# skovaka/UNCALLED

Measured on AMD Instinct MI355X. Metric: reads_mapped_per_sec, higher is better.
Workload: dtype u64+f32/f64; 1 GPU; E. coli 4.6 Mb synthetic ref (ecoli_syn seed 1), synthetic r9.4.1 reads (3600 bases ~ 32k samples, 10% off-target), all reference defaults; batches_in_flight=2, remapped_reads=0, parallelism=reads sharded over 1 GPU(s), index replicated

## Files before the change

### uncalled_amd/csrc/k_map.hip

```cpp
#include <hip/hip_runtime.h>

#include <type_traits>

#include "fm_dev.h"
#include "unc_dev_types.h"
#include "wave_prims.h"


#include "map_lds.h"
#include "map_sched.h"
#include "map_tracker.h"
#include "map_sort.h"
#include "map_sort_wide.h"

namespace unc {

__device__ __forceinline__ uint32_t float_orderable(float f) {
    uint32_t u = __float_as_uint(f);
    return (u & 0x80000000u) ? ~u : (u | 0x80000000u);
}

struct ChildHdr { uint32_t moves, meta; float seed_prob, last; uint64_t hist; };
__device__ __forceinline__ ChildHdr make_child(uint32_t pmoves, uint32_t pmeta, float last, float subc, uint64_t hist, uint64_t s, uint64_t e,
                                               uint32_t kmer, float prob, uint32_t move, uint32_t p_seed_len, float p_min_seed_prob,
// ... 12 lines not shown
    if (full) moves |= PATH_TAIL_MOVE;
    c.moves = moves;
    c.meta = kmer | (len << META_LEN_SHIFT) | (cstay << META_STAY_SHIFT) | (pmeta & META_SA_CHECKED) |
             ((!full && len == (uint32_t)SEED_LEN) ? META_FIRST_FULL : 0u);
    c.hist = move ? (hist & 0x3FFull) | ((((hist >> 10) << 2) | (kmer & 3u)) << 10) : hist;
    const uint32_t move_count = (uint32_t)__popc(moves);
    const bool seed_ok = len == p_seed_len && c.seed_prob >= p_min_seed_prob && s == e && (moves & 1u) == 1u &&
                         (float)(len - move_count) <= p_max_stay;
    key.a = key_len_bits ? ((((s << key_len_bits) | (e - s)) << 16) | child_idx) : ((s << KEY_LEN_BITS) | (e - s));
    key.b = ((uint64_t)float_orderable(c.seed_prob) << 32) | ((uint64_t)child_idx << 16) | (move_count << KEYB_MOVES_SHIFT) |
            (seed_ok ? KEYB_SEED_FLAG : 0u) | kmer;
    return c;
}

template <bool NARROW>
__device__ __forceinline__ void write_source(gptr_t buf, uint32_t idx, uint64_t s, uint64_t e, uint32_t kmer, float prob) {
    const uint32_t o = idx << PATH_SHIFT;
    const uint64_t r = NARROW ? (s | (e << 32)) : ((s << KEY_LEN_BITS) | (e - s));
    gst(buf, o, make_uint4((uint32_t)r, (uint32_t)(r >> 32), 1u, kmer | (1u << META_LEN_SHIFT)));
    gst(buf, o + 16u, make_uint4(__float_as_uint(prob), 0u, kmer, 0u));
}


#ifndef UNC_LB
#define UNC_LB 4
#endif

typedef const UNC_AS_CONST MapArgs *kargs_t;

struct WaveCtx {
    uint32_t event_i, n_parents, cur, n_surv_par;
    uint32_t tstatus;
    uint32_t nchild, n_seedp;
    uint32_t mixed;
    uint32_t kl;
    uint32_t scnt[6];
    uint32_t n_surv, n_src;
    uint32_t conf;
    uint32_t par_unsorted;
    uint32_t walked;
    uint32_t notes;
    uint32_t flags_save[NKMER / 32];
};
__shared__ WaveCtx s_w;
__shared__ Tracker s_T;
__shared__ uint64_t s_cyc[12];

__device__ __forceinline__ uint32_t ctx_get(const uint32_t &f) { return uniform32(f); }
#define CTX_SET(field, v) do { if (lane == 0) s_w.field = (v); } while (0)

#ifndef UNC_PROF_SORT
#define UNC_PROF_SORT 0
#endif
template <bool PROF> struct PhaseClock {
    uint64_t tk;
    __device__ __forceinline__ PhaseClock() : tk(PROF ? (uint64_t)clock64() : 0ull) {}
    __device__ __forceinline__ void reset() { if constexpr (PROF) tk = (uint64_t)clock64(); }
    __device__ __forceinline__ void end(int i, int lane) {
        if constexpr (PROF) {
            if ((UNC_PROF_SORT || UNC_DBG_SEED) && i >= 8) i = 1;
            const uint64_t tn = (uint64_t)clock64();
            if (lane == 0) s_cyc[i] += tn - tk;
            tk = tn;
        }
    }
};
#if UNC_PROF_SORT
struct SortClock {
    uint64_t tk;
    __device__ __forceinline__ SortClock() : tk((uint64_t)clock64()) {}
    __device__ __forceinline__ void end(int i, int lane) {
        const uint64_t tn = (uint64_t)clock64();
        if (lane == 0) { s_cyc[i] += tn - tk; s_cyc[2] -= tn - tk; }
        tk = tn;
    }
};
#else
struct SortClock { __device__ __forceinline__ void end(int, int) {} };
#endif

__device__ __forceinline__ TrackerMem tracker_mem(kargs_t A, gptr_t sb) {
    TrackerMem M;
    M.sb = sb; M.off_heads = A->sc.off_cl_dir; M.off_chunks = A->sc.off_cl_chunks;
    M.max_nodes = A->sc.max_clusters / 4 ? A->sc.max_clusters / 4 : 1u;
    M.n_buckets = A->ix.n_buckets; M.shift = A->ix.bucket_shift;
    M.pool.nodes = (gptr_t)A->pool.nodes;
    M.pool.q = A->pool.q; M.pool.cells = A->pool.cells; M.pool.cap_mask = A->pool.cap_mask;
    return M;
}

static __device__ __noinline__ void phase_P(kargs_t A_, float level, int lane) {
    const kargs_t A = uniform_ptr(A_);
    const UNC_AS_GLOBAL float4 *const model4 = (const UNC_AS_GLOBAL float4 *)A->ix.model4;
#pragma unroll 4
    for (int j = 0; j < NKMER / WAVE; ++j) {
        const uint32_t k = (uint32_t)j * WAVE + (uint32_t)lane;
        const float4 row = g_load(model4 + k);
        const float mu = row.x, v2 = row.y, ld = row.z;
        const float d = __fsub_rn(level, mu);
        const double q = -((double)d * (double)d) / (double)v2;
        s_probs[k] = (float)(q - (double)ld);
    }
    wave_sync();
}

struct FmView {
    const UNC_AS_GLOBAL uint32_t *bwt;
    const UNC_AS_GLOBAL uint32_t *fm32;
    const UNC_AS_GLOBAL uint64_t *sa, *sa_dense;
    const UNC_AS_CONST uint64_t *L2;
    uint64_t primary, seq_len;
};
__device__ __forceinline__ FmView fm_view(kargs_t A) {
// ... 252 lines not shown
        for (uint32_t l0 = 0; l0 < nwrite; l0 += WAVE) {
            const uint32_t li = l0 + (uint32_t)lane;
            if (li < nwrite) {
                const uint32_t d = s_cdesc[li];
                const uint32_t pl = d & 63u, type = (d >> 6) & 7u, ci = (pl << 2) | ((type - 1u) & 3u);
                const uint32_t pmt = s_pmeta[pl], pmv = s_pmoves[pl];
                const float last = s_plast[pl], subc = s_psubc[pl];
                const uint64_t hist = s_phist[pl];
                const uint32_t pk = pmt & META_KMER_MASK;
                Row cs, ce;
                uint32_t ck, mv;
                if (type == 0) { cs = s_pstart[pl]; ce = s_pend[pl]; ck = pk; mv = 0; }
                else {
                    const uint64_t pr = s_res[ci];
                    if constexpr (NARROW) { cs = (uint32_t)pr; ce = cs + (uint32_t)(pr >> 32) - 1u; }
                    else { cs = pr >> RES_BITS; ce = cs + (pr & ((1ull << RES_BITS) - 1ull)) - 1ull; }
                    ck = ((pk << 2) & KMASK) | (type - 1u); mv = 1;
                }
                SortKey key;
                const uint32_t gi = nchild + li;
                const ChildHdr c = make_child(pmv, pmt, last, subc, hist, cs, ce, ck, s_probs[ck], mv, p_seed_len, p_min_seed_prob, p_max_stay, gi, klb, key);
                const uint32_t co = chd_off + (gi << PATH_SHIFT);
                if constexpr (NARROW) gst(sb, co, make_uint4(cs, ce, c.moves, c.meta));
                else { const uint64_t r = (cs << KEY_LEN_BITS) | (ce - cs); gst(sb, co, make_uint4((uint32_t)r, (uint32_t)(r >> 32), c.moves, c.meta)); }
                gst(sb, co + 16u, make_uint4(__float_as_uint(c.last), __float_as_uint(subc), (uint32_t)c.hist, (uint32_t)(c.hist >> 32)));
                if constexpr (NARROW) {
                    const uint32_t run = (d >> 9) ? 5u : type;
                    gst(sb, str_off + run * run_bytes + ((uint32_t)s_ckpos[li] << 3), key.a);
                    gst(sb, info_off + (gi << 3), key.b);
                } else {
                    const bool csrc = base + pl >= n_surv_par;
                    const uint64_t wm = type == 0u ? wm0 : type == 1u ? wm1 : type == 2u ? wm2 : type == 3u ? wm3 : wm4;
                    const uint32_t ws = type == 0u ? ws0 : type == 1u ? ws1 : type == 2u ? ws2 : type == 3u ? ws3 : ws4;
                    const uint32_t kpos = csrc ? wsx + (li - w_src_cpos0) : ws + (uint32_t)__popcll(wm & ((1ull << pl) - 1ull));
                    gst(sb, str_off + (csrc ? 5u : type) * (run_bytes << 1) + (kpos << 4), key);
                }
            }
        }
        nchild += nwrite;
        wave_sync();
        clk.end(11, lane);
    }
    clk.end(1, lane);
    uint32_t tst = 0;
    if (n_seedp > max_seed_paths) { tst = UNC_READ_SEED_OVERFLOW; n_seedp = max_seed_paths; }
    if (lane == 0) {
        s_w.nchild = nchild; s_w.n_seedp = n_seedp; s_w.tstatus |= tst; s_w.par_unsorted = par_bad ? 1u : 0u;
        s_w.scnt[0] = scnt0; s_w.scnt[1] = scnt1; s_w.scnt[2] = scnt2; s_w.scnt[3] = scnt3; s_w.scnt[4] = scnt4; s_w.scnt[5] = scntx;
    }
    wave_sync();
    return c_nbr;
}

static __device__ __noinline__ void merge_walk(kargs_t A_, gptr_t sb_, KeyArr<1> KA_, KeyArr<4> KB_, int lane);
static __device__ __noinline__ void merge_walk_w(kargs_t A_, gptr_t sb_, KeyArr<1> KA_, KeyArr<4> KB_, int lane);

template <bool NARROW>
static __device__ __noinline__ void phase_S(kargs_t A_, gptr_t sb_, int lane) {
    const kargs_t A = uniform_ptr(A_);
    const gptr_t sb = uniform_ptr(sb_);
    const uint32_t n = ctx_get(s_w.nchild);
    const uint32_t max_paths = A->sc.max_paths;
    const uint32_t ukeys_off = A->sc.off_keys, skeys_off = A->sc.off_keys + A->sc.keys_cap * (uint32_t)sizeof(SortKey);
    UNC_AS_GLOBAL SortKey *const ukeys = reinterpret_cast<UNC_AS_GLOBAL SortKey *>(sb + ukeys_off);
    UNC_AS_GLOBAL SortKey *const skeys = reinterpret_cast<UNC_AS_GLOBAL SortKey *>(sb + skeys_off);
    uint32_t kl = NARROW ? A->ix.key_len_bits : 0u;
    if (lane == 0) { s_w.walked = 0u; s_w.mixed = 0u; }
    if constexpr (NARROW) {
        const uint32_t str_off = A->sc.off_streams, sk_off = skeys_off, run_bytes = max_paths << 3;
        uint32_t scnt0 = ctx_get(s_w.scnt[0]), scnt1 = ctx_get(s_w.scnt[1]), scnt2 = ctx_get(s_w.scnt[2]), scnt3 = ctx_get(s_w.scnt[3]),
                 scnt4 = ctx_get(s_w.scnt[4]), nx = ctx_get(s_w.scnt[5]);
#ifdef LANESIM
        {
            const uint32_t cnt[6] = {scnt0, scnt1, scnt2, scnt3, scnt4, nx};
            uint32_t tot = 0;
            for (uint32_t r = 0; r < 6; ++r) {
                tot += cnt[r];
                for (uint32_t i = (uint32_t)lane; i < cnt[r]; i += WAVE)
                    UNC_SIM_CHECK((gld<uint64_t>(sb, str_off + r * run_bytes + (i << 3)) & 0xFFFFu) < n);
            }
            UNC_SIM_CHECK(tot == n);
        }
#endif
        if (n > MERGE_MIN && !ctx_get(s_w.par_unsorted)) {
            const uint32_t x_off = str_off + 5u * run_bytes;
            uint32_t nviol = 0;
            SortClock sclk;
            if (scnt1 > 1 || scnt2 > 1 || scnt3 > 1 || scnt4 > 1) {
                const uint64_t v4 = repair_runs4(sb, str_off, run_bytes, scnt1, scnt2, scnt3, scnt4, x_off, nx, lane);
                const uint32_t v1 = (uint32_t)v4 & 0xFFFFu, v2 = (uint32_t)(v4 >> 16) & 0xFFFFu, v3 = (uint32_t)(v4 >> 32) & 0xFFFFu, v4r = (uint32_t)(v4 >> 48);
                nviol = v1 + v2 + v3 + v4r;
                if constexpr (MERGE_REPAIR) { scnt1 -= v1; scnt2 -= v2; scnt3 -= v3; scnt4 -= v4r; nx += nviol; }
            }
            wave_sync();
            sclk.end(8, lane);
            if (MERGE_REPAIR || nviol == 0) {
                if (nx > 1) {
                    KeyArr<6> KX;
#pragma unroll
                    for (int r = 0; r < 6; ++r) { KX.adj[r] = x_off; KX.cum[r] = 0; }
                    KX.n = nx;
                    sort_any64(sb, KX, x_off, lane);
                    wave_sync();
                }
                sclk.end(9, lane);
                KeyArr<4> KM;
                KM.cum[0] = 0; KM.cum[1] = scnt1; KM.cum[2] = scnt1 + scnt2; KM.cum[3] = scnt1 + scnt2 + scnt3;
                KM.n = KM.cum[3] + scnt4;
#pragma unroll
                for (uint32_t r = 0; r < 4; ++r) KM.adj[r] = str_off + (r + 1u) * run_bytes - (KM.cum[r] << 3);
                KeyArr<4> KB = KM;
                if (nx > 0) {
                    if (KM.n > 0) {
                        merge_runs<4, 1>(sb, KM, ka_single(x_off, nx), A->sc.off_tmp, lane, 0u);
                        wave_sync();
                        KB.adj[0] = A->sc.off_tmp;
                    } else KB.adj[0] = x_off;
                    KB.cum[1] = KB.cum[2] = KB.cum[3] = KB.n = KM.n + nx;
                    KB.adj[1] = KB.adj[2] = KB.adj[3] = KB.adj[0];
                }
                sclk.end(10, lane);
                merge_walk(A, sb, ka_single(str_off, scnt0), KB, lane);
                CTX_SET(kl, kl);
                CTX_SET(walked, 1u);
                wave_sync();
                sclk.end(11, lane);
                return;
            }
        }
        {
            KeyArr<6> K6;
            const uint32_t c[6] = {scnt0, scnt1, scnt2, scnt3, scnt4, nx};
            uint32_t cum = 0;
#pragma unroll
            for (uint32_t r = 0; r < 6; ++r) { K6.cum[r] = cum; K6.adj[r] = str_off + r * run_bytes - (cum << 3); cum += c[r]; }
            K6.n = cum;
            sort_any64(sb, K6, sk_off, lane);
        }
    }
    if constexpr (!NARROW) {
        const uint32_t str_off = A->sc.off_streams, run_bytes = max_paths << 4;
        uint32_t scnt0 = ctx_get(s_w.scnt[0]), scnt1 = ctx_get(s_w.scnt[1]), scnt2 = ctx_get(s_w.scnt[2]), scnt3 = ctx_get(s_w.scnt[3]),
                 scnt4 = ctx_get(s_w.scnt[4]), nx = ctx_get(s_w.scnt[5]);
        const uint32_t x_off = str_off + 5u * run_bytes;
        if (n > MERGE_MIN && !ctx_get(s_w.par_unsorted)) {
            if (scnt1 > 1) { const uint32_t v = repairw_run(sb, str_off + run_bytes, scnt1, x_off, nx, lane); scnt1 -= v; nx += v; }
            if (scnt2 > 1) { const uint32_t v = repairw_run(sb, str_off + 2u * run_bytes, scnt2, x_off, nx, lane); scnt2 -= v; nx += v; }
            if (scnt3 > 1) { const uint32_t v = repairw_run(sb, str_off + 3u * run_bytes, scnt3, x_off, nx, lane); scnt3 -= v; nx += v; }
            if (scnt4 > 1) { const uint32_t v = repairw_run(sb, str_off + 4u * run_bytes, scnt4, x_off, nx, lane); scnt4 -= v; nx += v; }
            wave_sync();
            uint32_t xs_off = x_off;
            if (nx > 1) {
                const UNC_AS_GLOBAL SortKey *const xin = reinterpret_cast<const UNC_AS_GLOBAL SortKey *>(sb + x_off);
                if (nx <= 64) sort_regs<1>(xin, skeys, nx, lane);
                else if (nx <= 128) sort_regs<2>(xin, skeys, nx, lane);
                else if (nx <= 256) sort_regs<4>(xin, skeys, nx, lane);
                else if (nx <= 512) sort_regs<8>(xin, skeys, nx, lane);
                else sort_hybrid(xin, skeys, nx, lane);
                xs_off = skeys_off;
                wave_sync();
            }
            KeyArr<4> KM;
            KM.cum[0] = 0; KM.cum[1] = scnt1; KM.cum[2] = scnt1 + scnt2; KM.cum[3] = scnt1 + scnt2 + scnt3;
            KM.n = KM.cum[3] + scnt4;
#pragma unroll
            for (uint32_t r = 0; r < 4; ++r) KM.adj[r] = str_off + (r + 1u) * run_bytes - (KM.cum[r] << 4);
            KeyArr<4> KB = KM;
            if (nx > 0) {
                if (KM.n > 0) {
                    mergew_runs<4, 1>(sb, KM, kaw_single(xs_off, nx), ukeys_off, lane);
                    wave_sync();
                    KB.adj[0] = ukeys_off;
                } else KB.adj[0] = xs_off;
                KB.cum[1] = KB.cum[2] = KB.cum[3] = KB.n = KM.n + nx;
                KB.adj[1] = KB.adj[2] = KB.adj[3] = KB.adj[0];
// ... 179 lines not shown
        kq0 = (uint32_t)lane < n ? k0 : ~0ull; kq1 = (uint32_t)lane + WAVE < n ? k1 : ~0ull;
        const uint32_t km0 = (uint32_t)(bq0 & META_KMER_MASK);
        krq = g_load(reinterpret_cast<const UNC_AS_GLOBAL u32x4_t *>(kmer_ranges2) + (s_probs[km0] >= source_prob ? km0 : 0u));
    }
    for (uint32_t base = 0; base < n; base += WAVE) {
        const uint32_t i = base + (uint32_t)lane;
        const bool have = i < n;
        const bool has_next = i + 1 < n;
        const uint32_t nv = n - base < WAVE ? n - base : WAVE;
        Row start, end, nstart;
        uint64_t sbw;
        uint32_t kmer, nkmer;
        bool dup;
        ulonglong2 krc = make_ulonglong2(1ull, 0ull);
        uint32_t kq2i = 0;
        if (kl) {
            const uint64_t ki = kq0, bi = bq0;
            uint64_t kn = (uint64_t)__shfl((unsigned long long)ki, (lane + 1) & 63);
            uint64_t bn = (uint64_t)__shfl((unsigned long long)bi, (lane + 1) & 63);
            const uint64_t kf = bcast64(kq1, 0), bf = bcast64(bq1, 0);
            if (lane == WAVE - 1) { kn = kf; bn = bf; }
            kq0 = kq1; bq0 = bq1;
            {
                const uint64_t k2 = skeys64[i + 2 * WAVE < n ? i + 2 * WAVE : n - 1u];
                kq1 = i + 2 * WAVE < n ? k2 : ~0ull;
                kq2i = (uint32_t)(k2 & 0xFFFFu);
            }
            u32x4_t kt = krq;
            mem_retire(kt);
            krc.x = ((uint64_t)kt.y << 32) | kt.x; krc.y = ((uint64_t)kt.w << 32) | kt.z;
            {
                const uint32_t kmn = (uint32_t)(bq0 & META_KMER_MASK);
                krq = g_load(reinterpret_cast<const UNC_AS_GLOBAL u32x4_t *>(kmer_ranges2) + (s_probs[kmn] >= source_prob ? kmn : 0u));
            }
            walk_decode_narrow<NARROW>(S, kl, ki, kn, bi, bn, have, has_next, nv, lane, start, end, nstart, kmer, nkmer, dup, sbw);
        } else {
            SortKey ki, kn;
            ki.a = ~0ull; ki.b = 0; kn.a = ~0ull; kn.b = ~0ull;
            if (have) ki = g_load(skeys + i);
            if (has_next) kn = g_load(skeys + i + 1);
            start = (Row)(ki.a >> KEY_LEN_BITS); end = start + (Row)(ki.a & KEY_LEN_MASK);
            nstart = (Row)(kn.a >> KEY_LEN_BITS);
            kmer = have ? (uint32_t)(ki.b & META_KMER_MASK) : NKMER + 1u;
            nkmer = has_next ? (uint32_t)(kn.b & META_KMER_MASK) : NKMER + 2u;
            dup = has_next && kn.a == ki.a;
            sbw = ki.b;
        }
        walk_core<NARROW>(C, S, have, has_next, start, end, nstart, kmer, nkmer, dup, sbw, kl != 0, krc, nv, lane);
        if (kl) bq1 = infow[kq2i];
    }
    walk_finish<NARROW>(C, S, lane);
}

static __device__ __noinline__ void merge_walk(kargs_t A_, gptr_t sb_, KeyArr<1> KA_, KeyArr<4> KB_, int lane) {
    const kargs_t A = uniform_ptr(A_);
    const gptr_t sb = uniform_ptr(sb_);
    uint64_t *const s_tile = s_e;
    const KeyArr<1> KA = ka_uniform(KA_);
    const KeyArr<4> KB = ka_uniform(KB_);
    const uint32_t n = KA.n + KB.n;
    const WalkConst<true> C = walk_const<true>(A, sb);
    WalkState<true> S;
    S.n_seedp = ctx_get(s_w.n_seedp);
    walk_begin_narrow(lane);
    const uint32_t kl = A->ix.key_len_bits;
    const float source_prob = C.source_prob;
    const UNC_AS_GLOBAL ulonglong2 *const kmer_ranges2 = (const UNC_AS_GLOBAL ulonglong2 *)A->ix.kmer_ranges;
    const UNC_AS_GLOBAL uint64_t *const infow = reinterpret_cast<const UNC_AS_GLOBAL uint64_t *>(sb + A->sc.off_info);
    uint32_t a0 = 0, b0 = 0;
    uint64_t pend_key = 0;
    bool have_pend = false, bad = false;
    for (uint32_t o0 = 0; o0 < n; o0 += MERGE_TILE) {
        const uint32_t d1 = o0 + MERGE_TILE < n ? o0 + MERGE_TILE : n;
        const bool last_tile = d1 == n;
        const uint32_t a1 = last_tile ? KA.n : merge_split(sb, KA, KB, d1, lane);
        const uint32_t b1 = d1 - a1;
        const uint32_t na = a1 - a0, nb = b1 - b0, tn = na + nb;
        stage_tile(sb, KA, KB, a0, b0, na, tn, s_tile, lane);
        wave_sync();
        const uint32_t d = (uint32_t)lane * MERGE_C < tn ? (uint32_t)lane * MERGE_C : tn;
        const uint32_t cnt = tn - d < MERGE_C ? tn - d : MERGE_C;
        uint32_t lo = d > nb ? d - nb : 0u, hi = d < na ? d : na;
        while (__any(lo < hi)) {
            if (lo < hi) {
                const uint32_t mid = (lo + hi) >> 1;
                if (s_tile[mslot(mid)] < s_tile[mslot(na + d - 1u - mid)]) lo = mid + 1u; else hi = mid;
            }
        }
        uint32_t ia = lo, ib = d - lo;
        uint64_t va = ia < na ? s_tile[mslot(ia)] : ~0ull, vb = ib < nb ? s_tile[mslot(na + ib)] : ~0ull;
        uint64_t o[MERGE_C];
#pragma unroll
        for (uint32_t c = 0; c < MERGE_C; ++c) {
            const bool ta = va < vb;
            o[c] = ta ? va : vb;
            if (ta) ++ia; else ++ib;
            const uint32_t idx = ta ? ia : na + ib;
            const bool ok = ta ? ia < na : ib < nb;
            uint64_t x = ~0ull;
            if (ok && c + 1u < cnt) x = s_tile[mslot(idx)];
            if (ta) va = x; else vb = x;
        }
        {
            uint64_t last = o[0];
            bool w = false;
#pragma unroll
            for (uint32_t c = 1; c < MERGE_C; ++c)
                if (c < cnt) { w = w || !(o[c] > last); last = o[c]; }
            uint64_t pl = (uint64_t)__shfl_up((unsigned long long)last, 1);
            if (lane == 0) pl = pend_key;
            if (cnt > 0 && !(o[0] > pl)) w = true;
            if (__any(w)) bad = true;
        }
        wave_sync();
#pragma unroll
        for (uint32_t c = 0; c < MERGE_C; ++c)
            if (c < cnt) s_tile[mslot(1u + d + c)] = o[c];
        if (lane == 0 && have_pend) s_tile[mslot(0)] = pend_key;
        wave_sync();
#ifdef LANESIM
        for (uint32_t q = 1u + (uint32_t)lane; q <= tn; q += WAVE) {
            const uint64_t kq = s_tile[mslot(q)];
            UNC_SIM_CHECK((kq & 0xFFFFu) < n);
            UNC_SIM_CHECK(((infow[kq & 0xFFFFu] >> 16) & 0xFFFFu) == (kq & 0xFFFFu));
        }
        wave_sync();
#endif
        const uint32_t p0 = have_pend ? 0u : 1u, p1 = last_tile ? tn + 1u : tn;
        uint64_t bq0, bq1;
        {
            const uint32_t pa = p0 + (uint32_t)lane, pb = pa + WAVE;
            bq0 = infow[s_tile[mslot(pa <= tn ? pa : tn)] & 0xFFFFu];
            bq1 = infow[s_tile[mslot(pb <= tn ? pb : tn)] & 0xFFFFu];
        }
        u32x4_t krq;
        {
            const uint32_t km0 = (uint32_t)(bq0 & META_KMER_MASK);
            krq = g_load(reinterpret_cast<const UNC_AS_GLOBAL u32x4_t *>(kmer_ranges2) + (s_probs[km0] >= source_prob ? km0 : 0u));
        }
        for (uint32_t base = p0; base < p1; base += WAVE) {
            const uint32_t p = base + (uint32_t)lane;
            const bool have = p < p1;
            const bool has_next = have && p < tn;
            const uint32_t nv = p1 - base < WAVE ? p1 - base : WAVE;
            const uint64_t bq2 = infow[s_tile[mslot(p + 2 * WAVE <= tn ? p + 2 * WAVE : tn)] & 0xFFFFu];
            const uint64_t ki = have ? s_tile[mslot(p)] : ~0ull, kn = has_next ? s_tile[mslot(p + 1u)] : ~0ull;
            const uint64_t bi = bq0;
            uint64_t bn = (uint64_t)__shfl((unsigned long long)bi, (lane + 1) & 63);
            const uint64_t bf = bcast64(bq1, 0);
            if (lane == WAVE - 1) bn = bf;
            bq0 = bq1;
            u32x4_t kt = krq;
            mem_retire(kt);
            ulonglong2 krc;
            krc.x = ((uint64_t)kt.y << 32) | kt.x; krc.y = ((uint64_t)kt.w << 32) | kt.z;
            {
                const uint32_t kmn = (uint32_t)(bq0 & META_KMER_MASK);
                krq = g_load(reinterpret_cast<const UNC_AS_GLOBAL u32x4_t *>(kmer_ranges2) + (s_probs[kmn] >= source_prob ? kmn : 0u));
            }
            uint32_t start, end, nstart, kmer, nkmer;
            uint64_t sbw;
            bool dup;
            walk_decode_narrow<true>(S, kl, ki, kn, bi, bn, have, has_next, nv, lane, start, end, nstart, kmer, nkmer, dup, sbw);
            walk_core<true>(C, S, have, has_next, start, end, nstart, kmer, nkmer, dup, sbw, true, krc, nv, lane);
            bq1 = bq2;
        }
        pend_key = uniform64(s_tile[mslot(tn)]);
        have_pend = true;
        a0 = a1; b0 = b1;
        wave_sync();
    }
    if (bad && lane == 0) s_w.tstatus |= UNC_READ_SORT_FAULT;
    walk_finish<true>(C, S, lane);
}

static __device__ __noinline__ void merge_walk_w(kargs_t A_, gptr_t sb_, KeyArr<1> KA_, KeyArr<4> KB_, int lane) {
    const kargs_t A = uniform_ptr(A_);
    const gptr_t sb = uniform_ptr(sb_);
    SortKey *const tile = reinterpret_cast<SortKey *>(s_e);
    const KeyArr<1> KA = ka_uniform(KA_);
    const KeyArr<4> KB = ka_uniform(KB_);
    const uint32_t n = KA.n + KB.n;
    const WalkConst<false> C = walk_const<false>(A, sb);
    WalkState<false> S;
    S.n_seedp = ctx_get(s_w.n_seedp);
    uint32_t a0 = 0, b0 = 0;
    SortKey pend_key; pend_key.a = 0; pend_key.b = 0;
    bool have_pend = false, bad = false;
    for (uint32_t o0 = 0; o0 < n; o0 += MERGEW_TILE) {
        const uint32_t d1 = o0 + MERGEW_TILE < n ? o0 + MERGEW_TILE : n;
        const bool last_tile = d1 == n;
        const uint32_t a1 = last_tile ? KA.n : mergew_split(sb, KA, KB, d1, lane);
        const uint32_t b1 = d1 - a1;
        const uint32_t na = a1 - a0, nb = b1 - b0, tn = na + nb;
        stagew_tile(sb, KA, KB, a0, b0, na, tn, tile, lane);
        wave_sync();
        SortKey o[MERGEW_C];
        uint32_t d, cnt;
        mergew_tile(tile, na, nb, lane, o, d, cnt);
        {
            SortKey last = o[0];
            bool w = false;
#pragma unroll
            for (uint32_t c = 1; c < MERGEW_C; ++c)
                if (c < cnt) { w = w || !wk_lt(last, o[c]); last = o[c]; }
            SortKey pl;
            pl.a = (uint64_t)__shfl_up((unsigned long long)last.a, 1); pl.b = (uint64_t)__shfl_up((unsigned long long)last.b, 1);
            if (lane == 0) pl = pend_key;
            if (cnt > 0 && !wk_lt(pl, o[0])) w = true;
            if (__any(w)) bad = true;
        }
        wave_sync();
#pragma unroll
        for (uint32_t c = 0; c < MERGEW_C; ++c)
            if (c < cnt) tile[1u + d + c] = o[c];
        if (lane == 0 && have_pend) tile[0] = pend_key;
        wave_sync();
        const uint32_t p0 = have_pend ? 0u : 1u, p1 = last_tile ? tn + 1u : tn;
        const UNC_AS_GLOBAL ulonglong2 *const kmer_ranges2 = (const UNC_AS_GLOBAL ulonglong2 *)A->ix.kmer_ranges;
        ulonglong2 krq;
        {
            const uint32_t pa = p0 + (uint32_t)lane;
            const uint32_t km0 = (uint32_t)(tile[pa <= tn ? pa : tn].b & META_KMER_MASK);
            krq = g_load(kmer_ranges2 + (s_probs[km0] >= C.source_prob ? km0 : 0u));
        }
// ... 1179 lines not shown
    else hipLaunchKernelGGL((k_map<false, false>), dim3(grid), dim3(WAVE), 0, st, a);
}
__global__ void k_sched_init(DevSched S) {
    const uint32_t t = blockIdx.x * blockDim.x + threadIdx.x, cap = S.cap_mask + 1u;
    const uint32_t part = t / cap, i = t % cap, spp = S.n_slots / S.n_parts;
    if (part < S.n_parts) {
        SchedCell f; f.seq = i < spp ? i + 1u : i; f.val = part * spp + i;
        S.free_cells[t] = f;
        SchedCell p; p.seq = i; p.val = 0;
        S.park_cells[t] = p;
    }
    if (t == 0) {
        SchedCtl c;
        memset(&c, 0, sizeof c);
        for (uint32_t q = 0; q < S.n_parts; ++q) c.freeq[q].tail = spp;
        *S.ctl = c;
    }
}
void launch_sched_init(const DevSched &S, hipStream_t st) {
    const uint32_t n = (S.cap_mask + 1u) * S.n_parts;
    hipLaunchKernelGGL(k_sched_init, dim3((n + 255) / 256), dim3(256), 0, st, S);
}
__global__ void k_xcd_probe(uint32_t *out) { if (threadIdx.x == 0) out[blockIdx.x] = xcd_id(); }
void launch_xcd_probe(uint32_t *out, uint32_t n_blocks, hipStream_t st) { hipLaunchKernelGGL(k_xcd_probe, dim3(n_blocks), dim3(64), 0, st, out); }
__global__ void k_pool_init(DevPool B) {
    const uint32_t i = blockIdx.x * blockDim.x + threadIdx.x, cap = B.cap_mask + 1u;
    if (i < cap) {
        SchedCell f; f.seq = i < B.n_chunks ? i + 1u : i; f.val = i;
        B.cells[i] = f;
    }
    if (i == 0) {
        PoolQueue q;
        memset(&q, 0, sizeof q);
        q.avail = (int32_t)B.n_chunks;
        q.tail = B.n_chunks;
        q.low_water = B.n_chunks;
        *B.q = q;
    }
}
void launch_pool_init(const DevPool &B, hipStream_t st) {
    const uint32_t cap = B.cap_mask + 1u;
    hipLaunchKernelGGL(k_pool_init, dim3((cap + 255) / 256), dim3(256), 0, st, B);
}
uint32_t map_kernel_waves_per_cu() { return 4 * UNC_LB; }
int map_kernel_attributes(bool narrow, bool profile, uint32_t *out4) {
    hipFuncAttributes a;
    const void *f = narrow ? (profile ? (const void *)k_map<true, true> : (const void *)k_map<false, true>)
                           : (profile ? (const void *)k_map<true, false> : (const void *)k_map<false, false>);
    const hipError_t e = hipFuncGetAttributes(&a, f);
    if (e != hipSuccess) return (int)e;
    out4[0] = (uint32_t)a.numRegs; out4[1] = (uint32_t)a.localSizeBytes; out4[2] = (uint32_t)a.sharedSizeBytes; out4[3] = (uint32_t)a.maxThreadsPerBlock;
    return 0;
}
}
```

### uncalled_amd/csrc/map_sort.h

```cpp
#pragma once

namespace unc {


__device__ __forceinline__ bool key_gt(uint64_t a1, uint64_t b1, uint64_t a2, uint64_t b2) {
    return a1 > a2 || (a1 == a2 && b1 > b2);
}

template <int E>
__device__ __forceinline__ void merge_stages(uint64_t (&a)[E], uint64_t (&b)[E], uint32_t base, uint32_t k, uint32_t j_from,
                                             int lane) {
    for (uint32_t j = j_from; j > 0; j >>= 1) {
        if (j >= (uint32_t)E) {
            const uint32_t d = j / (uint32_t)E;
            const bool lower = ((uint32_t)lane & d) == 0;
#pragma unroll
            for (int e = 0; e < E; ++e) {
                uint64_t pa = xor_lane64(a[e], d);
                uint64_t pb = xor_lane64(b[e], d);
                uint32_t p = base + (uint32_t)lane * E + (uint32_t)e;
                bool up = (p & k) == 0;
                bool want_min = lower == up;
                bool gt = key_gt(a[e], b[e], pa, pb);
                if (want_min ? gt : !gt) { a[e] = pa; b[e] = pb; }
// ... 289 lines not shown
static __device__ __noinline__ void sort_any64(gptr_t sb, KeyArr<6> K, uint32_t out_off, int lane) {
    const uint32_t n = uniform32(K.n);
    if (n <= 64) sort_regs64<1>(sb, K, out_off, lane);
    else if (n <= 128) sort_regs64<2>(sb, K, out_off, lane);
    else if (n <= 256) sort_regs64<4>(sb, K, out_off, lane);
    else if (n <= 512) sort_regs64<8>(sb, K, out_off, lane);
    else sort_hybrid64(sb, K, out_off, lane);
}

constexpr uint32_t MERGE_MIN = 256;
#ifndef UNC_MERGE_REPAIR
#define UNC_MERGE_REPAIR 1
#endif
constexpr bool MERGE_REPAIR = UNC_MERGE_REPAIR != 0;
constexpr uint32_t MERGE_C = 9;
constexpr uint32_t MERGE_TILE = MERGE_C * WAVE;
__device__ __forceinline__ uint32_t mslot(uint32_t i) { return i + (i >> 3); }
constexpr uint32_t MERGE_LDS_KEYS = MERGE_TILE + MERGE_TILE / 8 + 1;
static_assert(MERGE_LDS_KEYS <= S_E_WORDS && NKMER * 4 <= S_E_WORDS * 8, "merge tile / source list must fit the staging buffer");

constexpr uint32_t SPLIT_PROBES = 16;
template <int RA, int RB>
__device__ __forceinline__ uint32_t merge_split(cgptr_t sb, const KeyArr<RA> &A, const KeyArr<RB> &B, uint32_t d, int lane) {
    uint32_t lo = d > B.n ? d - B.n : 0u, hi = d < A.n ? d : A.n;
    while (lo < hi) {
        const uint32_t span = hi - lo, step = (span + SPLIT_PROBES - 1u) / SPLIT_PROBES;
        const uint32_t p = lo + (uint32_t)lane * step;
        bool less = false;
        if ((uint32_t)lane < SPLIT_PROBES && p < hi) less = ka_load(sb, A, p) < ka_load(sb, B, d - 1u - p);
        const uint32_t c = (uint32_t)__popcll(__ballot(less));
        const uint32_t nlo = c ? lo + (c - 1u) * step + 1u : lo;
        const uint32_t nhi = lo + c * step < hi ? lo + c * step : hi;
        lo = nlo; hi = c ? nhi : lo;
    }
    return lo;
}

template <int RA, int RB>
__device__ __forceinline__ void stage_tile(cgptr_t sb, const KeyArr<RA> &A, const KeyArr<RB> &B, uint32_t a0, uint32_t b0, uint32_t na, uint32_t tn,
                                           uint64_t *s_tile, int lane) {
    uint64_t v[MERGE_C];
#pragma unroll
    for (uint32_t c = 0; c < MERGE_C; ++c) {
        const uint32_t i0 = (uint32_t)lane + c * WAVE, i = i0 < tn ? i0 : tn - 1u;
        const uint32_t ja = a0 + i, jb = b0 + (i - na);
        const uint32_t off = i < na ? ka_adj(A, ja) + (ja << 3) : ka_adj(B, jb) + (jb << 3);
        v[c] = gld<uint64_t>(sb, off);
    }
#pragma unroll
    for (uint32_t c = 0; c < MERGE_C; ++c) {
        const uint32_t i = (uint32_t)lane + c * WAVE;
        if (i < tn) s_tile[mslot(i)] = v[c];
    }
}

template <int RA, int RB>
static __device__ __noinline__ uint32_t merge_runs(gptr_t sb_, KeyArr<RA> A_, KeyArr<RB> B_, uint32_t out_off_, int lane, uint32_t verify_) {
    const gptr_t sb = uniform_ptr(sb_);
    uint64_t *const s_tile = s_e;
    const KeyArr<RA> A = ka_uniform(A_);
    const KeyArr<RB> B = ka_uniform(B_);
    const uint32_t out_off = uniform32(out_off_), verify = uniform32(verify_);
    const uint32_t n = A.n + B.n;
    uint32_t a0 = 0, b0 = 0;
    uint64_t prev_last = 0;
    bool bad = false;
    for (uint32_t o0 = 0; o0 < n; o0 += MERGE_TILE) {
        const uint32_t d1 = o0 + MERGE_TILE < n ? o0 + MERGE_TILE : n;
        const uint32_t a1 = d1 == n ? A.n : merge_split(sb, A, B, d1, lane);
        const uint32_t b1 = d1 - a1;
        const uint32_t na = a1 - a0, nb = b1 - b0, tn = na + nb;
        stage_tile(sb, A, B, a0, b0, na, tn, s_tile, lane);
        wave_sync();
        const uint32_t d = (uint32_t)lane * MERGE_C < tn ? (uint32_t)lane * MERGE_C : tn;
        const uint32_t cnt = tn - d < MERGE_C ? tn - d : MERGE_C;
        uint32_t lo = d > nb ? d - nb : 0u, hi = d < na ? d : na;
        while (__any(lo < hi)) {
            if (lo < hi) {
                const uint32_t mid = (lo + hi) >> 1;
                if (s_tile[mslot(mid)] < s_tile[mslot(na + d - 1u - mid)]) lo = mid + 1u; else hi = mid;
            }
        }
        uint32_t ia = lo, ib = d - lo;
        uint64_t va = ia < na ? s_tile[mslot(ia)] : ~0ull, vb = ib < nb ? s_tile[mslot(na + ib)] : ~0ull;
        uint64_t o[MERGE_C];
#pragma unroll
        for (uint32_t c = 0; c < MERGE_C; ++c) {
            const bool ta = va < vb;
            o[c] = ta ? va : vb;
            if (ta) ++ia; else ++ib;
            const uint32_t idx = ta ? ia : na + ib;
            const bool ok = ta ? ia < na : ib < nb;
            uint64_t x = ~0ull;
            if (ok && c + 1u < cnt) x = s_tile[mslot(idx)];
            if (ta) va = x; else vb = x;
        }
        wave_sync();
#pragma unroll
        for (uint32_t c = 0; c < MERGE_C; ++c)
            if (c < cnt) s_tile[mslot(d + c)] = o[c];
        wave_sync();
#pragma unroll
        for (uint32_t c = 0; c < MERGE_C; ++c) {
            const uint32_t i = (uint32_t)lane + c * WAVE;
            if (i < tn) gst(sb, out_off + ((o0 + i) << 3), s_tile[mslot(i)]);
        }
// ... 114 lines not shown
```

Measured before the change: 25170 reads/s.

## Fold small extra-key run into merge-walk as a three-way in-register merge

When the unsorted extra-key run has at most a wavefront's worth of keys, it is now loaded into registers, sorted with a single in-wave bitonic sort, and merged tile-by-tile into the merge walk. Previously it was sorted in global scratch and merged into the four repaired runs through a separate merge_runs pass into temporary storage. This removes a global sort and a full merge pass over the four runs for the common case. The cost is a second in-tile merge and extra LDS syncs on tiles that absorb extra keys, plus some added register pressure in merge_walk. Larger extra runs keep the old path.

```diff
diff --git a/uncalled_amd/csrc/k_map.hip b/uncalled_amd/csrc/k_map.hip
--- a/uncalled_amd/csrc/k_map.hip
+++ b/uncalled_amd/csrc/k_map.hip
@@ -88,13 +88,16 @@
 #ifndef UNC_PROF_SORT
 #define UNC_PROF_SORT 0
 #endif
+#ifndef UNC_DBG_NX
+#define UNC_DBG_NX 0
+#endif
 template <bool PROF> struct PhaseClock {
     uint64_t tk;
     __device__ __forceinline__ PhaseClock() : tk(PROF ? (uint64_t)clock64() : 0ull) {}
     __device__ __forceinline__ void reset() { if constexpr (PROF) tk = (uint64_t)clock64(); }
     __device__ __forceinline__ void end(int i, int lane) {
         if constexpr (PROF) {
-            if ((UNC_PROF_SORT || UNC_DBG_SEED) && i >= 8) i = 1;
+            if ((UNC_PROF_SORT || UNC_DBG_NX || UNC_DBG_SEED) && i >= 8) i = 1;
             const uint64_t tn = (uint64_t)clock64();
             if (lane == 0) s_cyc[i] += tn - tk;
             tk = tn;
@@ -453,7 +456,14 @@
     return c_nbr;
 }
 
-static __device__ __noinline__ void merge_walk(kargs_t A_, gptr_t sb_, KeyArr<1> KA_, KeyArr<4> KB_, int lane);
+static __device__ __noinline__ void merge_walk(kargs_t A_, gptr_t sb_, KeyArr<1> KA_, KeyArr<4> KB_, uint32_t x_off_, uint32_t nx_, int lane);
+
+#ifdef LANESIM
+extern "C" { unsigned long long unc_sim_merge3_count = 0, unc_sim_merge2_count = 0, unc_sim_merge_nx_hist[MERGE_XCAP + 3] = {0}; }
+#define UNC_SIM_COUNT(c) do { if (lane == 0) __atomic_fetch_add(&(c), 1ull, __ATOMIC_RELAXED); } while (0)
+#else
+#define UNC_SIM_COUNT(c) ((void)0)
+#endif
 static __device__ __noinline__ void merge_walk_w(kargs_t A_, gptr_t sb_, KeyArr<1> KA_, KeyArr<4> KB_, int lane);
 
 template <bool NARROW>
@@ -495,23 +505,30 @@
             }
             wave_sync();
             sclk.end(8, lane);
+#if UNC_DBG_NX
+            if (lane == 0 && (MERGE_REPAIR || nviol == 0)) { s_cyc[8] += 1u; s_cyc[9] += nx <= 64u; s_cyc[10] += nx <= 128u; s_cyc[11] += nviol; }
+#endif
             if (MERGE_REPAIR || nviol == 0) {
-                if (nx > 1) {
+                KeyArr<4> KM;
+                KM.cum[0] = 0; KM.cum[1] = scnt1; KM.cum[2] = scnt1 + scnt2; KM.cum[3] = scnt1 + scnt2 + scnt3;
+                KM.n = KM.cum[3] + scnt4;
+#pragma unroll
+                for (uint32_t r = 0; r < 4; ++r) KM.adj[r] = str_off + (r + 1u) * run_bytes - (KM.cum[r] << 3);
+                if (nx <= MERGE_XCAP) {
+                    UNC_SIM_COUNT(unc_sim_merge3_count);
+                    UNC_SIM_COUNT(unc_sim_merge_nx_hist[nx]);
+                    merge_walk(A, sb, ka_single(str_off, scnt0), KM, x_off, nx, lane);
+                } else {
+                    UNC_SIM_COUNT(unc_sim_merge2_count);
+                    UNC_SIM_COUNT(unc_sim_merge_nx_hist[nx < MERGE_XCAP + 2u ? nx : MERGE_XCAP + 2u]);
                     KeyArr<6> KX;
 #pragma unroll
                     for (int r = 0; r < 6; ++r) { KX.adj[r] = x_off; KX.cum[r] = 0; }
                     KX.n = nx;
                     sort_any64(sb, KX, x_off, lane);
                     wave_sync();
-                }
-                sclk.end(9, lane);
-                KeyArr<4> KM;
-                KM.cum[0] = 0; KM.cum[1] = scnt1; KM.cum[2] = scnt1 + scnt2; KM.cum[3] = scnt1 + scnt2 + scnt3;
-                KM.n = KM.cum[3] + scnt4;
-#pragma unroll
-                for (uint32_t r = 0; r < 4; ++r) KM.adj[r] = str_off + (r + 1u) * run_bytes - (KM.cum[r] << 3);
-                KeyArr<4> KB = KM;
-                if (nx > 0) {
+                    sclk.end(9, lane);
+                    KeyArr<4> KB = KM;
                     if (KM.n > 0) {
                         merge_runs<4, 1>(sb, KM, ka_single(x_off, nx), A->sc.off_tmp, lane, 0u);
                         wave_sync();
@@ -519,9 +536,9 @@
                     } else KB.adj[0] = x_off;
                     KB.cum[1] = KB.cum[2] = KB.cum[3] = KB.n = KM.n + nx;
                     KB.adj[1] = KB.adj[2] = KB.adj[3] = KB.adj[0];
-                }
-                sclk.end(10, lane);
-                merge_walk(A, sb, ka_single(str_off, scnt0), KB, lane);
+                    sclk.end(10, lane);
+                    merge_walk(A, sb, ka_single(str_off, scnt0), KB, x_off, 0u, lane);
+                }
                 CTX_SET(kl, kl);
                 CTX_SET(walked, 1u);
                 wave_sync();
@@ -807,13 +824,15 @@
     walk_finish<NARROW>(C, S, lane);
 }
 
-static __device__ __noinline__ void merge_walk(kargs_t A_, gptr_t sb_, KeyArr<1> KA_, KeyArr<4> KB_, int lane) {
+static __device__ __noinline__ void merge_walk(kargs_t A_, gptr_t sb_, KeyArr<1> KA_, KeyArr<4> KB_, uint32_t x_off_, uint32_t nx_, int lane) {
     const kargs_t A = uniform_ptr(A_);
     const gptr_t sb = uniform_ptr(sb_);
     uint64_t *const s_tile = s_e;
     const KeyArr<1> KA = ka_uniform(KA_);
     const KeyArr<4> KB = ka_uniform(KB_);
-    const uint32_t n = KA.n + KB.n;
+    const uint32_t nx = uniform32(nx_);
+    const uint32_t n2 = KA.n + KB.n;
+    const uint64_t xk = merge3_load_x(sb, uniform32(x_off_), nx, lane);
     const WalkConst<true> C = walk_const<true>(A, sb);
     WalkState<true> S;
     S.n_seedp = ctx_get(s_w.n_seedp);
@@ -822,61 +841,15 @@
     const float source_prob = C.source_prob;
     const UNC_AS_GLOBAL ulonglong2 *const kmer_ranges2 = (const UNC_AS_GLOBAL ulonglong2 *)A->ix.kmer_ranges;
     const UNC_AS_GLOBAL uint64_t *const infow = reinterpret_cast<const UNC_AS_GLOBAL uint64_t *>(sb + A->sc.off_info);
-    uint32_t a0 = 0, b0 = 0;
-    uint64_t pend_key = 0;
-    bool have_pend = false, bad = false;
-    for (uint32_t o0 = 0; o0 < n; o0 += MERGE_TILE) {
-        const uint32_t d1 = o0 + MERGE_TILE < n ? o0 + MERGE_TILE : n;
-        const bool last_tile = d1 == n;
-        const uint32_t a1 = last_tile ? KA.n : merge_split(sb, KA, KB, d1, lane);
-        const uint32_t b1 = d1 - a1;
-        const uint32_t na = a1 - a0, nb = b1 - b0, tn = na + nb;
-        stage_tile(sb, KA, KB, a0, b0, na, tn, s_tile, lane);
-        wave_sync();
-        const uint32_t d = (uint32_t)lane * MERGE_C < tn ? (uint32_t)lane * MERGE_C : tn;
-        const uint32_t cnt = tn - d < MERGE_C ? tn - d : MERGE_C;
-        uint32_t lo = d > nb ? d - nb : 0u, hi = d < na ? d : na;
-        while (__any(lo < hi)) {
-            if (lo < hi) {
-                const uint32_t mid = (lo + hi) >> 1;
-                if (s_tile[mslot(mid)] < s_tile[mslot(na + d - 1u - mid)]) lo = mid + 1u; else hi = mid;
-            }
-        }
-        uint32_t ia = lo, ib = d - lo;
-        uint64_t va = ia < na ? s_tile[mslot(ia)] : ~0ull, vb = ib < nb ? s_tile[mslot(na + ib)] : ~0ull;
-        uint64_t o[MERGE_C];
-#pragma unroll
-        for (uint32_t c = 0; c < MERGE_C; ++c) {
-            const bool ta = va < vb;
-            o[c] = ta ? va : vb;
-            if (ta) ++ia; else ++ib;
-            const uint32_t idx = ta ? ia : na + ib;
-            const bool ok = ta ? ia < na : ib < nb;
-            uint64_t x = ~0ull;
-            if (ok && c + 1u < cnt) x = s_tile[mslot(idx)];
-            if (ta) va = x; else vb = x;
-        }
-        {
-            uint64_t last = o[0];
-            bool w = false;
-#pragma unroll
-            for (uint32_t c = 1; c < MERGE_C; ++c)
-                if (c < cnt) { w = w || !(o[c] > last); last = o[c]; }
-            uint64_t pl = (uint64_t)__shfl_up((unsigned long long)last, 1);
-            if (lane == 0) pl = pend_key;
-            if (cnt > 0 && !(o[0] > pl)) w = true;
-            if (__any(w)) bad = true;
-        }
-        wave_sync();
-#pragma unroll
-        for (uint32_t c = 0; c < MERGE_C; ++c)
-            if (c < cnt) s_tile[mslot(1u + d + c)] = o[c];
-        if (lane == 0 && have_pend) s_tile[mslot(0)] = pend_key;
-        wave_sync();
+    Merge3 M;
+    while (M.o0 < n2) {
+        const bool have_pend = M.have_pend;
+        const uint32_t tn = merge3_tile(sb, KA, KB, nx, xk, M, s_tile, lane);
+        const bool last_tile = M.last_tile;
 #ifdef LANESIM
         for (uint32_t q = 1u + (uint32_t)lane; q <= tn; q += WAVE) {
             const uint64_t kq = s_tile[mslot(q)];
-            UNC_SIM_CHECK((kq & 0xFFFFu) < n);
+            UNC_SIM_CHECK((kq & 0xFFFFu) < n2 + nx);
             UNC_SIM_CHECK(((infow[kq & 0xFFFFu] >> 16) & 0xFFFFu) == (kq & 0xFFFFu));
         }
         wave_sync();
@@ -920,12 +893,10 @@
             walk_core<true>(C, S, have, has_next, start, end, nstart, kmer, nkmer, dup, sbw, true, krc, nv, lane);
             bq1 = bq2;
         }
-        pend_key = uniform64(s_tile[mslot(tn)]);
-        have_pend = true;
-        a0 = a1; b0 = b1;
-        wave_sync();
-    }
-    if (bad && lane == 0) s_w.tstatus |= UNC_READ_SORT_FAULT;
+        merge3_done(M, tn, s_tile);
+    }
+    UNC_SIM_CHECK(M.xc == nx);
+    if (M.bad && lane == 0) s_w.tstatus |= UNC_READ_SORT_FAULT;
     walk_finish<true>(C, S, lane);
 }
 
@@ -2211,4 +2182,37 @@
     out4[0] = (uint32_t)a.numRegs; out4[1] = (uint32_t)a.localSizeBytes; out4[2] = (uint32_t)a.sharedSizeBytes; out4[3] = (uint32_t)a.maxThreadsPerBlock;
     return 0;
 }
-}
+
+#ifdef LANESIM
+__global__ void k_sim_merge3(char *buf, uint32_t run_keys, const uint32_t *cnt, uint64_t *out, uint32_t *tiles) {
+    const int lane = lane_id();
+    const gptr_t sb = (gptr_t)buf;
+    const uint32_t run_bytes = run_keys << 3, nx = cnt[5];
+    KeyArr<4> KM;
+    KM.cum[0] = 0; KM.cum[1] = cnt[1]; KM.cum[2] = cnt[1] + cnt[2]; KM.cum[3] = cnt[1] + cnt[2] + cnt[3];
+    KM.n = KM.cum[3] + cnt[4];
+    for (uint32_t r = 0; r < 4; ++r) KM.adj[r] = (r + 1u) * run_bytes - (KM.cum[r] << 3);
+    const KeyArr<1> KA = ka_single(0u, cnt[0]);
+    const uint64_t xk = merge3_load_x(sb, 5u * run_bytes, nx, lane);
+    Merge3 M;
+    uint32_t nt = 0, pos = 0;
+    bool pend_ok = true;
+    while (M.o0 < KA.n + KM.n) {
+        const bool have_pend = M.have_pend;
+        const uint64_t pend = M.pend_key;
+        const uint32_t tn = merge3_tile(sb, KA, KM, nx, xk, M, s_e, lane);
+        for (uint32_t q = 1u + (uint32_t)lane; q <= tn; q += WAVE) out[pos + q - 1u] = s_e[mslot(q)];
+        if (have_pend && s_e[mslot(0)] != pend) pend_ok = false;
+        if (lane == 0) tiles[++nt] = tn;
+        pos += tn;
+        merge3_done(M, tn, s_e);
+    }
+    if (lane == 0) tiles[0] = nt | ((M.bad || !pend_ok || M.xc != nx) ? 0u : 1u << 31);
+}
+#endif
+}
+#ifdef LANESIM
+extern "C" void unc_sim_merge3(void *buf, uint32_t run_keys, const uint32_t *cnt, uint64_t *out, uint32_t *tiles) {
+    hipLaunchKernelGGL(unc::k_sim_merge3, dim3(1), dim3(64), 0, 0, (char *)buf, run_keys, cnt, out, tiles);
+}
+#endif
diff --git a/uncalled_amd/csrc/map_sort.h b/uncalled_amd/csrc/map_sort.h
--- a/uncalled_amd/csrc/map_sort.h
+++ b/uncalled_amd/csrc/map_sort.h
@@ -365,6 +365,102 @@
         const uint32_t i = (uint32_t)lane + c * WAVE;
         if (i < tn) s_tile[mslot(i)] = v[c];
     }
+}
+
+__device__ __forceinline__ void tile_merge(const uint64_t *s_tile, uint32_t na, uint32_t nb, uint32_t d, uint32_t cnt, uint64_t (&o)[MERGE_C]) {
+    uint32_t lo = d > nb ? d - nb : 0u, hi = d < na ? d : na;
+    while (__any(lo < hi)) {
+        if (lo < hi) {
+            const uint32_t mid = (lo + hi) >> 1;
+            if (s_tile[mslot(mid)] < s_tile[mslot(na + d - 1u - mid)]) lo = mid + 1u; else hi = mid;
+        }
+    }
+    uint32_t ia = lo, ib = d - lo;
+    uint64_t va = ia < na ? s_tile[mslot(ia)] : ~0ull, vb = ib < nb ? s_tile[mslot(na + ib)] : ~0ull;
+#pragma unroll
+    for (uint32_t c = 0; c < MERGE_C; ++c) {
+        const bool ta = va < vb;
+        o[c] = ta ? va : vb;
+        if (ta) ++ia; else ++ib;
+        const uint32_t idx = ta ? ia : na + ib;
+        const bool ok = ta ? ia < na : ib < nb;
+        uint64_t x = ~0ull;
+        if (ok && c + 1u < cnt) x = s_tile[mslot(idx)];
+        if (ta) va = x; else vb = x;
+    }
+}
+
+constexpr uint32_t MERGE_XCAP = WAVE;
+struct Merge3 {
+    uint32_t a0 = 0, b0 = 0, o0 = 0;
+    uint32_t xc = 0;
+    uint64_t pend_key = 0;
+    bool have_pend = false, last_tile = false, bad = false;
+};
+template <int RA, int RB>
+__device__ __forceinline__ uint32_t merge3_tile(cgptr_t sb, const KeyArr<RA> &A, const KeyArr<RB> &B, uint32_t nx, uint64_t xk, Merge3 &M,
+                                                uint64_t *s_tile, int lane) {
+    const uint32_t n2 = A.n + B.n, adv = MERGE_TILE - (nx - M.xc);
+    const uint32_t d1 = M.o0 + adv < n2 ? M.o0 + adv : n2;
+    M.last_tile = d1 == n2;
+    const uint32_t a1 = M.last_tile ? A.n : merge_split(sb, A, B, d1, lane);
+    const uint32_t b1 = d1 - a1;
+    const uint32_t na = a1 - M.a0, nb = b1 - M.b0, tn2 = na + nb;
+    stage_tile(sb, A, B, M.a0, M.b0, na, tn2, s_tile, lane);
+    wave_sync();
+    uint32_t nxt = 0;
+    if (M.xc < nx) {
+        const uint64_t ta = s_tile[mslot(na ? na - 1u : 0u)], tb = s_tile[mslot(tn2 - 1u)];
+        const uint64_t tmax = ta > tb ? ta : tb;
+        nxt = (uint32_t)__popcll(__ballot((uint32_t)lane >= M.xc && (uint32_t)lane < nx && (M.last_tile || xk < tmax)));
+    }
+    uint32_t tn = tn2;
+    uint32_t d = (uint32_t)lane * MERGE_C < tn ? (uint32_t)lane * MERGE_C : tn;
+    uint32_t cnt = tn - d < MERGE_C ? tn - d : MERGE_C;
+    uint64_t o[MERGE_C];
+    tile_merge(s_tile, na, nb, d, cnt, o);
+    if (nxt) {
+        wave_sync();
+#pragma unroll
+        for (uint32_t c = 0; c < MERGE_C; ++c)
+            if (c < cnt) s_tile[mslot(d + c)] = o[c];
+        if ((uint32_t)lane >= M.xc && (uint32_t)lane < M.xc + nxt) s_tile[mslot(tn2 + (uint32_t)lane - M.xc)] = xk;
+        wave_sync();
+        tn = tn2 + nxt;
+        d = (uint32_t)lane * MERGE_C < tn ? (uint32_t)lane * MERGE_C : tn;
+        cnt = tn - d < MERGE_C ? tn - d : MERGE_C;
+        tile_merge(s_tile, tn2, nxt, d, cnt, o);
+    }
+    {
+        uint64_t last = o[0];
+        bool w = false;
+#pragma unroll
+        for (uint32_t c = 1; c < MERGE_C; ++c)
+            if (c < cnt) { w = w || !(o[c] > last); last = o[c]; }
+        uint64_t pl = (uint64_t)__shfl_up((unsigned long long)last, 1);
+        if (lane == 0) pl = M.pend_key;
+        if (cnt > 0 && !(o[0] > pl)) w = true;
+        if (__any(w)) M.bad = true;
+    }
+    wave_sync();
+#pragma unroll
+    for (uint32_t c = 0; c < MERGE_C; ++c)
+        if (c < cnt) s_tile[mslot(1u + d + c)] = o[c];
+    if (lane == 0 && M.have_pend) s_tile[mslot(0)] = M.pend_key;
+    wave_sync();
+    M.a0 = a1; M.b0 = b1; M.o0 = d1; M.xc += nxt;
+    return tn;
+}
+__device__ __forceinline__ void merge3_done(Merge3 &M, uint32_t tn, const uint64_t *s_tile) {
+    M.pend_key = uniform64(s_tile[mslot(tn)]);
+    M.have_pend = true;
+    wave_sync();
+}
+__device__ __forceinline__ uint64_t merge3_load_x(cgptr_t sb, uint32_t x_off, uint32_t nx, int lane) {
+    const uint64_t k = gld<uint64_t>(sb, x_off + (((uint32_t)lane < nx ? (uint32_t)lane : 0u) << 3));
+    uint64_t a[1] = {(uint32_t)lane < nx ? k : ~0ull};
+    if (nx > 1) block_sort64<1>(a, lane);
+    return a[0];
 }
 
 template <int RA, int RB>
```

Result: slower. 23180 reads/s (-7.9%).
